# bowang-lab/BioReason

Hardware: AMD Instinct MI355X
Metric: GRPO samples/sec (NT-500M+Qwen3-1.7B, DNA 2x1024, prompt 2180, gen 256) (higher is better)
Workload: dtype bf16

## Files before the change

bioreason_amd/csrc/k_lora.hip:

```cpp
#include "bra_device.h"
#include "bra_api_internal.h"
#include "bra_lora_plan.h"

namespace bra {

struct LoraDownArgs {
    const bf16_t* x; long ldx;
    const bf16_t* A; long lda;
    bf16_t* t; long ldt;
    int M, K, R;
    float alpha;
    DropCfg d;
    int nb_live;
    int steps_per;
    float* part;
};

template <int RB, int NL, int TR = 32, int NT = NL>
__global__ __launch_bounds__(256) void lora_down_drop_kernel(LoraDownArgs g) {
    static_assert(TR == 8 || TR == 16 || TR == 32 || TR == 64 || TR == 128, "adapter ranks with dropout");
    static_assert(NL == (NT * TR + 31) / 32 && NL <= RB && NT <= 4, "live blocks = the blocks the targets cover");
    constexpr int KS = 128, XP = KS + 8;
    constexpr int XS_ELEMS = 2 * 32 * XP, AS_ELEMS = 2 * 32 * NL * XP;
    constexpr int RED_BYTES = 3 * NL * 64 * 16 * 4, STAGE_BYTES = (XS_ELEMS + AS_ELEMS) * 2;
    __shared__ __attribute__((aligned(16))) char lds[STAGE_BYTES > RED_BYTES ? STAGE_BYTES : RED_BYTES];
    bf16_t* xs = reinterpret_cast<bf16_t*>(lds);
    bf16_t* as = xs + XS_ELEMS;
    float* red = reinterpret_cast<float*>(lds);
    const int tid = (int)threadIdx.x, lane = tid & 63, wave = tid >> 6, h = lane >> 5;
    const int m0 = (int)blockIdx.x * 32;
    const int nstep = (g.K + KS - 1) / KS;
    const u32x4 zero4 = {0u, 0u, 0u, 0u};
    u32x4 rx[2], ra[2 * NL];
    auto issue = [&](int s) {
#pragma unroll
        for (int i = 0; i < 2; ++i) {
            const int c = tid + 256 * i, row = c >> 4, k = KS * s + 8 * (c & 15);
            int m = m0 + row; m = m < g.M ? m : g.M - 1;
            rx[i] = ld16(g.x + (long)m * g.ldx + (k < g.K ? k : 0));
        }
#pragma unroll
        for (int i = 0; i < 2 * NL; ++i) {
            const int c = tid + 256 * i, row = c >> 4, k = KS * s + 8 * (c & 15);
            ra[i] = ld16(g.A + (long)(row < g.R ? row : g.R - 1) * g.lda + (k < g.K ? k : 0));
        }
    };
    auto commit = [&](int buf, int s) {
#pragma unroll
        for (int i = 0; i < 2; ++i) {
            const int c = tid + 256 * i, k = KS * s + 8 * (c & 15);
            st16(&xs[buf * 32 * XP + (c >> 4) * XP + 8 * (c & 15)], k < g.K ? rx[i] : zero4);
        }
#pragma unroll
        for (int i = 0; i < 2 * NL; ++i) {
            const int c = tid + 256 * i, row = c >> 4, k = KS * s + 8 * (c & 15);
            st16(&as[buf * 32 * NL * XP + (c >> 4) * XP + 8 * (c & 15)], (k < g.K && row < g.R) ? ra[i] : zero4);
        }
    };
    f32x16 acc[NL];
#pragma unroll
    for (int rb = 0; rb < NL; ++rb)
#pragma unroll
        for (int q = 0; q < 16; ++q) acc[rb][q] = 0.f;
    const int s_lo = (int)blockIdx.y * g.steps_per;
    const int s_hi = s_lo + g.steps_per < nstep ? s_lo + g.steps_per : nstep;
    issue(s_lo); commit(s_lo & 1, s_lo);
    __syncthreads();
    const int mrow = m0 + (lane & 31);
    for (int s = s_lo; s < s_hi; ++s) {
        const int buf = s & 1;
        issue(s + 1 < s_hi ? s + 1 : s);
        sched_fence();
        const int lrow = opaque_i(lane & 31);
#pragma unroll
        for (int k2 = 0; k2 < 2; ++k2) {
            const int kk = 2 * wave + k2;
            const u32x4 xf = ld16(&xs[buf * 32 * XP + lrow * XP + 16 * kk + 8 * h]);
            const uint32_t e0 = (uint32_t)mrow * (uint32_t)g.K + (uint32_t)(KS * s + 16 * kk + 8 * h);
            if constexpr (TR == 32) {
#pragma unroll
                for (int rb = 0; rb < NL; ++rb) {
                    const u32x4 af = drop_apply8(xf, g.d.seed[rb], e0, g.d.thr16, g.d.inv_keep);
                    const u32x4 bf = ld16(&as[buf * 32 * NL * XP + (32 * rb + lrow) * XP + 16 * kk + 8 * h]);
                    acc[rb] = mfma_32x32x16(af, bf, acc[rb]);
                }
            } else if constexpr (TR > 32) {
#pragma unroll
                for (int jt = 0; jt < NT; ++jt) {
                    const u32x4 af = drop_apply8(xf, g.d.seed[jt], e0, g.d.thr16, g.d.inv_keep);
#pragma unroll
                    for (int b = 0; b < TR / 32; ++b) {
                        const int rb = jt * (TR / 32) + b;
                        const u32x4 bf = ld16(&as[buf * 32 * NL * XP + (32 * rb + lrow) * XP + 16 * kk + 8 * h]);
                        acc[rb] = mfma_32x32x16(af, bf, acc[rb]);
                    }
                }
            } else {
#pragma unroll
                for (int jt = 0; jt < NT; ++jt) {
                    const int rb = jt * TR / 32;
                    const u32x4 af = drop_apply8(xf, g.d.seed[jt], e0, g.d.thr16, g.d.inv_keep);
                    const u32x4 bf = ld16(&as[buf * 32 * NL * XP + (32 * rb + lrow) * XP + 16 * kk + 8 * h]);
                    acc[rb] = mfma_32x32x16(af, lrow / TR == jt % (32 / TR) ? bf : zero4, acc[rb]);
                }
            }
        }
        if (s + 1 < s_hi) commit(buf ^ 1, s + 1);
        __syncthreads();
    }
    if (wave != 0) {
#pragma unroll
        for (int rb = 0; rb < NL; ++rb)
#pragma unroll
            for (int q = 0; q < 16; ++q) red[(((wave - 1) * NL + rb) * 64 + lane) * 16 + q] = acc[rb][q];
    }
    __syncthreads();
    if (wave != 0) return;
    float* const pbase = g.part ? g.part + ((long)blockIdx.y * g.M + m0 + 4 * h) * g.R + (lane & 31) : nullptr;
    bf16_t* const tbase = g.t ? g.t + (long)(m0 + 4 * h) * g.ldt + (lane & 31) : nullptr;
#pragma unroll
    for (int rb = 0; rb < RB; ++rb) {
        const int r = 32 * rb + (lane & 31);
#pragma unroll
        for (int q = 0; q < 16; ++q) {
            const int mq = (q & 3) + 8 * (q >> 2);
            const int m = m0 + mq + 4 * h;
            float v = 0.f;
            if (rb < NL) {
                v = acc[rb < NL ? rb : 0][q];
#pragma unroll
                for (int w = 0; w < 3; ++w) v += red[((w * NL + (rb < NL ? rb : 0)) * 64 + lane) * 16 + q];
            }
            if (m < g.M && r < g.R) {
                if (g.part) pbase[(long)mq * g.R + 32 * rb] = v;
                else tbase[(long)mq * g.ldt + 32 * rb] = f2bf(g.alpha * v);
            }
        }
    }
}

__global__ __launch_bounds__(256) void lora_partial_reduce_kernel(const float* part, int ks, long MR, int R, float alpha, bf16_t* t, long ldt) {
    const long i4 = ((long)blockIdx.x * 256 + threadIdx.x) * 4;
    if (i4 >= MR) return;
    float a0 = 0.f, a1 = 0.f, a2 = 0.f, a3 = 0.f;
    for (int k = 0; k < ks; ++k) {
        const f32x4 v = *reinterpret_cast<const f32x4*>(part + (long)k * MR + i4);
        a0 += v[0]; a1 += v[1]; a2 += v[2]; a3 += v[3];
    }
    const long m = i4 / R;
    const int r = (int)(i4 - m * R);
    bf16_t* o = t + m * ldt + r;
    o[0] = f2bf(alpha * a0); o[1] = f2bf(alpha * a1); o[2] = f2bf(alpha * a2); o[3] = f2bf(alpha * a3);
}

struct LoraUpArgs {
    const bf16_t* dts; long ldd;
    const bf16_t* AT; long ldat;
    bf16_t* out; long ldo;
    int M, K, R;
    int k_chunk;
    DropCfg d;
    int nb_live;
};

template <int RB, int NL, int TR = 32, int NT = NL>
__global__ __launch_bounds__(256) void lora_up_drop_kernel(LoraUpArgs g) {
    constexpr int NC = TR == 32 ? 2 * NL : (NT * TR + 15) / 16;
    const u32x4 zero4 = {0u, 0u, 0u, 0u};
    const int lane = lane_id(), wave = (int)threadIdx.x >> 6, h = lane >> 5;
    const int m_base = ((int)blockIdx.x * 4 + wave) * 32;
    if (m_base >= g.M) return;
    int mr = m_base + (lane & 31); mr = mr < g.M ? mr : g.M - 1;
    u32x4 df[NC];
#pragma unroll
    for (int c = 0; c < NC; ++c) df[c] = ld16(g.dts + (long)mr * g.ldd + 16 * c + 8 * h);
    uint32_t rowbase[8];
    {
        const uint32_t odd0 = (uint32_t)lane & 1u;
#pragma unroll
        for (int i = 0; i < 8; ++i) {
            const int q = (int)(8 * odd0) + i;
            rowbase[i] = (uint32_t)(m_base + (q & 3) + 8 * (q >> 2) + 4 * h) * (uint32_t)g.K;
        }
    }
    const int k_lo = (int)blockIdx.y * g.k_chunk;
    int k_hi = k_lo + g.k_chunk; k_hi = k_hi < g.K ? k_hi : g.K;
    constexpr int UP_SP = 64 + 8;
    __shared__ __attribute__((aligned(16))) bf16_t stage[4][32 * UP_SP];
    bf16_t* sw = stage[wave];
    const bool vec_ok = !(g.ldo & 7) && !((size_t)g.out & 15) && !(k_lo & 7);
    for (int k0 = k_lo; k0 < k_hi; k0 += 32) {
        const int kc = k0 + (lane & 31);
        const int kr = kc < g.K ? kc : g.K - 1;
        u32x4 af[NC];
#pragma unroll
        for (int c = 0; c < NC; ++c) af[c] = ld16(g.AT + (long)kr * g.ldat + 16 * c + 8 * h);
        float o[16];
#pragma unroll
        for (int q = 0; q < 16; ++q) o[q] = 0.f;
        const uint32_t odd = (uint32_t)kr & 1u;
        const uint32_t fsh = odd ? 17u : 1u;
#pragma unroll
        for (int rb = 0; rb < NT; ++rb) {
            f32x16 acc;
#pragma unroll
            for (int q = 0; q < 16; ++q) acc[q] = 0.f;
            if constexpr (TR >= 16) {
#pragma unroll
                for (int c = rb * (TR / 16); c < (rb + 1) * (TR / 16); ++c) acc = mfma_32x32x16(df[c], af[c], acc);
            } else {
                acc = mfma_32x32x16(h == rb % 2 ? df[rb / 2] : zero4, af[rb / 2], acc);
            }
            uint32_t hh[16];
#pragma unroll
            for (int i = 0; i < 8; ++i) {
                const uint32_t mine = drop_hash(g.d.seed[rb], (rowbase[i] + (uint32_t)kr) >> 1);
                const uint32_t other = lane_swap1(mine);
                hh[i] = odd ? other : mine;
                hh[8 + i] = odd ? mine : other;
            }
#pragma unroll
            for (int q = 0; q < 16; ++q) o[q] += ((hh[q] >> fsh) & 0x7fffu) >= g.d.thr16 ? acc[q] : 0.f;
        }
        const int side = ((k0 - k_lo) >> 5) & 1;
#pragma unroll
        for (int q = 0; q < 16; ++q)
            sw[((q & 3) + 8 * (q >> 2) + 4 * h) * UP_SP + 32 * side + (lane & 31)] = kc < g.K ? f2bf(o[q] * g.d.inv_keep) : (bf16_t)0;
        if (side == 1 || k0 + 32 >= k_hi) {
            wave_lds_sync();
            const int kf = k0 - 32 * side;
            const int ncol = 32 * (side + 1);
#pragma unroll
            for (int j = 0; j < 4; ++j) {
                const int row = 8 * j + (lane >> 3), c8 = 8 * (lane & 7);
                const int m = m_base + row;
                const u32x4 v = ld16(&sw[row * UP_SP + c8]);
                if (m < g.M && c8 < ncol) {
                    bf16_t* op = g.out + (long)m * g.ldo + kf + c8;
                    if (vec_ok && kf + c8 + 8 <= g.K) st16(op, v);
                    else {
                        const bf16_t* e = reinterpret_cast<const bf16_t*>(&v);
                        for (int i = 0; i < 8; ++i) if (kf + c8 + i < g.K) op[i] = e[i];
                    }
                }
            }
            wave_lds_sync();
        }
    }
}

__global__ __launch_bounds__(256) void dropout_mask_kernel(uint8_t* out, long n, uint32_t seed, uint32_t thr16) {
    for (long i = (long)blockIdx.x * 256 + threadIdx.x; i < n; i += (long)gridDim.x * 256)
        out[i] = drop_keep1(seed, (uint32_t)i, thr16) ? 1 : 0;
}

}

using namespace bra;

extern "C" int bra_lora_down_splitk_plan(int M, int K) {
    const int gx = (M + 31) / 32, nstep = (K + 127) / 128;
    if (gx >= 192) return nstep >= 32 ? 4 : 1;
    if (gx <= 0 || nstep < 6) return 1;
    int want = 512 / gx, cap = nstep / 3;
    int ks = want < cap ? want : cap;
    if (ks < 2) return 1;
    const int per = (nstep + ks - 1) / ks;
    return (nstep + per - 1) / per;
}

extern "C" int bra_lora_down_drop(const void* x, long ldx, const void* A, long lda, void* t, long ldt, int M, int K, int R,
                                  float alpha, float p, unsigned s0, unsigned s1, unsigned s2, unsigned s3, int r, int nt,
                                  float* part, int ksplit, void* stream) {
    if (M == 0) return 0;
    if (!x || !A || !t || M < 0 || K <= 0 || K % 8 || ldx % 8 || lda % 8 || !lora_drop_ok(p, M, K, r, nt, R)) return BRA_ERR_ARG;
    if (ksplit <= 1) part = nullptr;
    else if (!part || ksplit > (K + 127) / 128 || ldt % 4) return BRA_ERR_ARG;
    const unsigned seeds[4] = {s0, s1, s2, s3};
    const int nstep = (K + 127) / 128;
    const int per = part ? (nstep + ksplit - 1) / ksplit : nstep;
    const int ny = part ? (nstep + per - 1) / per : 1;
    const dim3 grid((M + 31) / 32, ny);
    bra_stream_t st = (bra_stream_t)stream;
    return lora_for_slices(r, nt, R, [&](const LoraSlice& s) {
        float* const ps = part ? part + (long)ksplit * M * s.c0 : nullptr;
        bf16_t* const ts = (bf16_t*)t + s.c0;
        LoraDownArgs g = {(const bf16_t*)x, ldx, (const bf16_t*)A + (long)s.c0 * lda, lda, ts, ldt, M, K, s.Rs, alpha,
                          make_cfg(p, seeds + s.j0, s.nts), 0, per, ps};
#define BRA_LD(C_, RB_, NL_, TR_, NT_) if (C_) BRA_LAUNCH((lora_down_drop_kernel<RB_, NL_, TR_, NT_>), grid, dim3(256), 0, st, g); else
        BRA_LORA_ROWS(BRA_LD) return BRA_ERR_ARG;
#undef BRA_LD
        if (part) {
            const long MR = (long)M * s.Rs;
            BRA_LAUNCH(lora_partial_reduce_kernel, dim3((unsigned)((MR / 4 + 255) / 256)), dim3(256), 0, st, (const float*)ps, ny, MR, s.Rs,
                       alpha, ts, ldt);
        }
        return BRA_LAUNCH_STATUS();
    });
}

extern "C" int bra_lora_up_drop(const void* dts, long ldd, const void* AT, long ldat, void* out, long ldo, int M, int K, int R,
                                float p, unsigned s0, unsigned s1, unsigned s2, unsigned s3, int r, int nt, void* stream) {
    if (M == 0) return 0;
    if (!dts || !AT || !out || M < 0 || K <= 0 || ldd % 8 || ldat % 8 || !lora_drop_ok(p, M, K, r, nt, R)) return BRA_ERR_ARG;
    const int mblk = (M + 127) / 128;
    int splits = (1024 + mblk - 1) / mblk;
    int k_chunk = ((K + splits - 1) / splits + 31) / 32 * 32;
    k_chunk = k_chunk < 128 ? 128 : k_chunk;
    const unsigned seeds[4] = {s0, s1, s2, s3};
    LoraUpArgs g = {(const bf16_t*)dts, ldd, (const bf16_t*)AT, ldat, (bf16_t*)out, ldo, M, K, R, k_chunk, make_cfg(p, seeds, nt), 0};
    const dim3 grid(mblk, (K + k_chunk - 1) / k_chunk);
    bra_stream_t st = (bra_stream_t)stream;
#define BRA_LU(RB_, NL_, TR_, NT_) BRA_LAUNCH((lora_up_drop_kernel<RB_, NL_, TR_, NT_>), grid, dim3(256), 0, st, g)
#define BRA_LUR(TR_, NT_) BRA_LU((NT_ * TR_ + 63) / 64 * 2, (NT_ * TR_ + 31) / 32, TR_, NT_)
#define BRA_LUR3(TR_) do { if (nt == 1) BRA_LUR(TR_, 1); else if (nt == 2) BRA_LUR(TR_, 2); else BRA_LUR(TR_, 3); } while (0)
    if (r == 32 && R == 32) BRA_LU(1, 1, 32, 1);
    else if (r == 32 && R == 64) { if (nt == 1) BRA_LU(2, 1, 32, 1); else BRA_LU(2, 2, 32, 2); }
    else if (r == 32 && nt == 3) BRA_LU(4, 3, 32, 3);
    else if (r == 32) BRA_LU(4, 4, 32, 4);
    else if (r == 8) BRA_LUR3(8);
    else if (r == 16) BRA_LUR3(16);
    else if (r == 64) BRA_LUR3(64);
    else BRA_LUR3(128);
#undef BRA_LUR3
#undef BRA_LUR
#undef BRA_LU
    return BRA_LAUNCH_STATUS();
}

extern "C" int bra_dropout_mask(void* out, int M, int K, float p, unsigned seed, void* stream) {
    if (M <= 0 || K <= 0) return 0;
    if (!out || !(p >= 0.f && p < 1.f) || (long)M * K >= (1l << 32)) return BRA_ERR_ARG;
    const long n = (long)M * K;
    long grid = (n + 255) / 256; grid = grid > 4096 ? 4096 : grid;
    BRA_LAUNCH(dropout_mask_kernel, dim3((unsigned)grid), dim3(256), 0, (bra_stream_t)stream, (uint8_t*)out, n, (uint32_t)seed,
               drop_threshold(p));
    return BRA_LAUNCH_STATUS();
}
```

bioreason_amd/ops.py:

```python
from __future__ import annotations

import math
import os
from typing import Optional, Tuple

import torch

from ._lib import current_stream, get_lib

BF16 = torch.bfloat16


def _ld(t: torch.Tensor) -> int:
    assert t.stride(-1) == 1, "last dim must be contiguous"
    return t.stride(-2) if t.dim() >= 2 else t.shape[-1]


def _rows(t: torch.Tensor) -> int:
    return t.numel() // t.shape[-1]


def _as2d(t: torch.Tensor) -> torch.Tensor:
    return t.reshape(-1, t.shape[-1]) if t.dim() != 2 else t


def gemm_nt(
    a: torch.Tensor,
    b: torch.Tensor,
    *,
    a2: Optional[torch.Tensor] = None,
    b2: Optional[torch.Tensor] = None,
    bias: Optional[torch.Tensor] = None,
    res: Optional[torch.Tensor] = None,
    out: Optional[torch.Tensor] = None,
    alpha: float = 1.0,
    out_f32: bool = False,
    accumulate: bool = False,
) -> torch.Tensor:
    a = _as2d(a)
    M, K = a.shape
    N = b.shape[0]
    assert b.shape[1] == K and a.dtype == BF16 and b.dtype == BF16
    K2 = 0
    if a2 is not None:
        a2 = _as2d(a2)
        K2 = a2.shape[1]
        assert b2 is not None and b2.shape == (N, K2) and a2.shape[0] == M
    if out is None:
        out = torch.empty((M, N), dtype=torch.float32 if out_f32 else BF16, device=a.device)
    else:
        assert out.shape == (M, N) and out.dtype == (torch.float32 if out_f32 else BF16)
    if res is not None:
        res = _as2d(res)
        assert res.shape == (M, N) and res.dtype == BF16
    prof = GEMM_PROFILE
    timed = prof is not None and a.is_cuda and prof.wants(M, N, K, K2)
    if timed:
        e0 = torch.cuda.Event(enable_timing=True)
        e0.record()
    get_lib().call(
        "bra_gemm_bf16_nt", a, _ld(a), b, _ld(b), a2, _ld(a2) if a2 is not None else 0, b2,
        _ld(b2) if b2 is not None else 0, K2, out, _ld(out), M, N, K, alpha, bias, res,
        _ld(res) if res is not None else 0, int(out_f32), int(accumulate), current_stream(a),
    )
    if timed:
        e1 = torch.cuda.Event(enable_timing=True)
        e1.record()
        nbytes = 2.0 * (M * K + N * K + (M + N) * K2 + (M * N if res is not None else 0)) + M * N * (4.0 if out_f32 else 2.0)
        prof.records.append((2.0 * M * N * (K + K2), e0, e1, nbytes, (M, N, K, K2, res is not None)))
    return out


class GemmProfile:

    def __init__(self, min_m: int = 1024, dominant_only: bool = True):
        self.min_m = min_m
        self.dominant_only = dominant_only
        self.records = []

    def wants(self, M: int, N: int, K: int, K2: int) -> bool:
        if not self.dominant_only:
            return M >= self.min_m
        if K % 64 or K2 % 64:
            return False
        t = ((M + 255) // 256) * ((N + 255) // 256)
        rounds = (t + 255) // 256
        if t >= 140 and (t <= 256 or 100 * t >= 75 * rounds * 256):
            return True
        if ((M + 255) // 256) * ((N + 127) // 128) >= 128:
            return True
        return ((M + 127) // 128) * ((N + 127) // 128) >= 128

    def summary(self):
        torch.cuda.synchronize()
        fl = sum(r[0] for r in self.records)
        ms = sum(r[1].elapsed_time(r[2]) for r in self.records)
        n = len(self.records)
        by = sum(r[3] for r in self.records)
        return {"launches": n, "flops": fl, "ms": ms, "avg_launch_ms": ms / max(n, 1), "tflops": fl / max(ms, 1e-9) / 1e9,
                "flops_per_launch": fl / max(n, 1), "bytes_per_launch": by / max(n, 1)}


def gemm_profile_by_shape(prof: "GemmProfile"):
    torch.cuda.synchronize()
    agg = {}
    for r in prof.records:
        a = agg.setdefault(r[4], [0, 0.0, 0.0])
        a[0] += 1
        a[1] += r[1].elapsed_time(r[2])
        a[2] += r[0]
    return sorted(((k, n, ms, fl / max(ms, 1e-9) / 1e9) for k, (n, ms, fl) in agg.items()), key=lambda t: -t[2])


GEMM_PROFILE: Optional[GemmProfile] = None


def gemm_nt_splitk(a: torch.Tensor, b: torch.Tensor, out: torch.Tensor, alpha: float = 1.0, split_k: int = 0) -> torch.Tensor:
    M, K = a.shape
    N = b.shape[0]
    assert b.shape[1] == K and out.shape == (M, N) and out.dtype == torch.float32
    if split_k <= 0:
        tiles = ((M + 127) // 128) * ((N + 127) // 128)
        split_k = max(1, min(K // 256 if K >= 256 else 1, (512 + tiles - 1) // tiles))
    get_lib().call("bra_gemm_bf16_nt_splitk", a, _ld(a), b, _ld(b), out, _ld(out), M, N, K, alpha, split_k, current_stream(a))
    return out


def wgrad_tn(y: torch.Tensor, t: torch.Tensor, out: torch.Tensor, transposed_out: bool = False, alpha: float = 1.0,
             m_chunk: int = 0, drop=None, rank: int = 32) -> torch.Tensor:
    M, N = y.shape
    R = t.shape[1]
    assert t.shape[0] == M and out.dtype == torch.float32 and out.shape == ((R, N) if transposed_out else (N, R))
    c_sn, c_sr = (1, _ld(out)) if transposed_out else (_ld(out), 1)
    if drop is not None:
        get_lib().call("bra_wgrad_tn_drop", y, _ld(y), t, _ld(t), out, c_sn, c_sr, M, N, R, alpha, m_chunk, drop[0],
                       *_group(drop[1], rank, R), current_stream(y))
        return out
    get_lib().call("bra_wgrad_tn", y, _ld(y), t, _ld(t), out, c_sn, c_sr, M, N, R, alpha, m_chunk, current_stream(y))
    return out


LORA_DROP_RANKS = (8, 16, 32, 64, 128)


def _group(seeds, rank, R):
    if rank not in LORA_DROP_RANKS:
        raise NotImplementedError(f"LoRA dropout is built for adapter ranks {list(LORA_DROP_RANKS)}, not r = {rank}")
    if rank == 32:
        seeds = seeds[:max(R // 32, 1)]
    elif not 1 <= len(seeds) <= 3:
        raise ValueError(f"a fused LoRA group has 1 to 3 targets, got {len(seeds)} seeds")
    s = [int(x) & 0xFFFFFFFF for x in seeds]
    return (*(s + [0, 0, 0, 0])[:4], rank, len(s))


def dropout_mask(M: int, K: int, p: float, seed: int, device) -> torch.Tensor:
    out = torch.empty((M, K), dtype=torch.uint8, device=device)
    get_lib().call("bra_dropout_mask", out, M, K, p, int(seed) & 0xFFFFFFFF, current_stream(out))
    return out


LORA_DOWN_SPLITK = os.environ.get("BRA_LORA_SPLITK", "1") != "0"


def lora_down_drop(x: torch.Tensor, A: torch.Tensor, alpha: float, p: float, seeds, rank: int = 32) -> torch.Tensor:
    M, K = x.shape
    R = A.shape[0]
    t = torch.empty((M, R), dtype=BF16, device=x.device)
    lib = get_lib()
    ks = int(lib._dll.bra_lora_down_splitk_plan(int(M), int(K))) if LORA_DOWN_SPLITK else 1
    part = torch.empty((ks, M, R), dtype=torch.float32, device=x.device) if ks > 1 else None
    lib.call("bra_lora_down_drop", x, _ld(x), A, _ld(A), t, _ld(t), M, K, R, alpha, p, *_group(seeds, rank, R), part, ks,
             current_stream(x))
    return t


def lora_up_drop(dts: torch.Tensor, AT: torch.Tensor, p: float, seeds, rank: int = 32) -> torch.Tensor:
    M, R = dts.shape
    K = AT.shape[0]
    out = torch.empty((M, K), dtype=BF16, device=dts.device)
    get_lib().call("bra_lora_up_drop", dts, _ld(dts), AT, _ld(AT), out, _ld(out), M, K, R, p, *_group(seeds, rank, R),
                   current_stream(dts))
    return out


def lmhead_logprob(h: torch.Tensor, emb: torch.Tensor, tgt: torch.Tensor) -> Tuple[torch.Tensor, torch.Tensor]:
    M, K = h.shape
    V = emb.shape[0]
    nchunk = (V + 63) // 64
    dev = h.device
    pm = torch.empty((M, nchunk), dtype=torch.float32, device=dev)
    ps = torch.empty((M, nchunk), dtype=torch.float32, device=dev)
    tl = torch.zeros((M,), dtype=torch.float32, device=dev)
    lse = torch.empty((M,), dtype=torch.float32, device=dev)
    logp = torch.empty((M,), dtype=torch.float32, device=dev)
    st = current_stream(h)
    lib = get_lib()
    lib.call("bra_lmhead_lse_partials", h, _ld(h), emb, _ld(emb), M, V, K, tgt, pm, ps, tl, st)
    lib.call("bra_lse_merge", pm, ps, tl, lse, logp, M, nchunk, st)
    return logp, lse


def lmhead_dlogits(h: torch.Tensor, emb: torch.Tensor, tgt: torch.Tensor, lse: torch.Tensor, coef: torch.Tensor) -> torch.Tensor:
    M, K = h.shape
    V = emb.shape[0]
    out = torch.empty((M, V), dtype=BF16, device=h.device)
    get_lib().call("bra_lmhead_dlogits", h, _ld(h), emb, _ld(emb), M, V, K, tgt, lse, coef, out, _ld(out), current_stream(h))
    return out


def rmsnorm_fwd(x: torch.Tensor, w: torch.Tensor, eps: float) -> torch.Tensor:
    x2 = _as2d(x)
    y = torch.empty_like(x2)
    get_lib().call("bra_rmsnorm_fwd", x2, _ld(x2), w, y, _ld(y), None, x2.shape[0], x2.shape[1], eps, current_stream(x))
    return y.view(x.shape)


def rmsnorm_bwd(dy: torch.Tensor, x: torch.Tensor, w: torch.Tensor, eps: float, dres: Optional[torch.Tensor] = None) -> torch.Tensor:
    x2, dy2 = _as2d(x), _as2d(dy)
    dx = torch.empty_like(x2)
    d2 = _as2d(dres) if dres is not None else None
    get_lib().call("bra_rmsnorm_bwd", dy2, _ld(dy2), x2, _ld(x2), w, d2, _ld(d2) if d2 is not None else 0, dx, _ld(dx),
                   x2.shape[0], x2.shape[1], eps, current_stream(x))
    return dx.view(x.shape)


def layernorm_fwd(x: torch.Tensor, w: torch.Tensor, b: torch.Tensor, eps: float) -> torch.Tensor:
    x2 = _as2d(x)
    y = torch.empty_like(x2)
    get_lib().call("bra_layernorm_fwd", x2, _ld(x2), w, b, y, _ld(y), x2.shape[0], x2.shape[1], eps, current_stream(x))
    return y.view(x.shape)


def gemm_swiglu(x: torch.Tensor, W: torch.Tensor, a2: Optional[torch.Tensor] = None, b2: Optional[torch.Tensor] = None) -> Optional[torch.Tensor]:
    M, K = x.shape
    F = W.shape[0] // 2
    K2 = a2.shape[1] if a2 is not None else 0
    if M <= 16 or K % 64 or K2 % 64 or F % 128 or W.shape[0] != 2 * F:
        return None
    act = torch.empty((M, F), dtype=BF16, device=x.device)
    rc = get_lib().call_rc("bra_gemm_swiglu_bf16_nt", x, _ld(x), W, _ld(W), a2, _ld(a2) if a2 is not None else 0, b2,
                           _ld(b2) if b2 is not None else 0, K2, act, _ld(act), M, F, K, 1.0, current_stream(x))
    return None if rc != 0 else act


def swiglu_fwd(gu: torch.Tensor) -> torch.Tensor:
    gu2 = _as2d(gu)
    F = gu2.shape[1] // 2
    act = torch.empty((gu2.shape[0], F), dtype=BF16, device=gu.device)
    get_lib().call("bra_swiglu_fwd", gu2, _ld(gu2), act, _ld(act), gu2.shape[0], F, current_stream(gu))
    return act


def swiglu_bwd(gu: torch.Tensor, dact: torch.Tensor) -> torch.Tensor:
    gu2, d2 = _as2d(gu), _as2d(dact)
    F = gu2.shape[1] // 2
    dgu = torch.empty_like(gu2)
    get_lib().call("bra_swiglu_bwd", gu2, _ld(gu2), d2, _ld(d2), dgu, _ld(dgu), gu2.shape[0], F, current_stream(gu))
    return dgu


def _bsh_strides(t: torch.Tensor) -> Tuple[int, int, int]:
    assert t.dim() == 4 and t.stride(3) == 1
    return t.stride(0), t.stride(1), t.stride(2)


def qk_norm_rope_fwd(qkv, qw, kw, cosT, sinT, pos, S, Hq, Hkv, hd, eps, qscale, q, k, v, s_off=0):
    T = qkv.shape[0]
    get_lib().call("bra_qk_norm_rope_fwd", qkv, _ld(qkv), qw, kw, cosT, sinT, pos, T, S, Hq, Hkv, hd, eps, qscale,
                   q, *_bsh_strides(q), k, *_bsh_strides(k), v, *_bsh_strides(v), s_off, current_stream(qkv))


def qk_norm_rope_bwd(qkv, qw, kw, cosT, sinT, pos, S, Hq, Hkv, hd, eps, qscale, dq, dk, dv):
    T = qkv.shape[0]
    dqkv = torch.empty_like(qkv)
    get_lib().call("bra_qk_norm_rope_bwd", qkv, _ld(qkv), qw, kw, cosT, sinT, pos, T, S, Hq, Hkv, hd, eps, qscale,
                   dq, *_bsh_strides(dq), dk, *_bsh_strides(dk), dv, *_bsh_strides(dv), dqkv, _ld(dqkv), current_stream(qkv))
    return dqkv


def pad64(n: int) -> int:
    return (n + 63) // 64 * 64


def head_transpose(x: torch.Tensor) -> torch.Tensor:
    B, S, H, hd = x.shape
    out = torch.empty((B, H, hd, pad64(S)), dtype=BF16, device=x.device)
    sb, ss, sh = _bsh_strides(x)
    get_lib().call("bra_head_transpose", x, sb, ss, sh, out, out.stride(0), out.stride(1), out.stride(2), B, S, H, hd, current_stream(x))
    return out


def attn_fwd(q, k, vt, kmask, causal: bool, scale: float, q_off: Optional[int] = None, need_lse: bool = True,
             out: Optional[torch.Tensor] = None, nsplit: Optional[int] = None):
    B, Sq, Hq, hd = q.shape
    Sk, Hkv = k.shape[1], k.shape[2]
    if q_off is None:
        q_off = Sk - Sq
    o = out if out is not None else torch.empty((B, Sq, Hq, hd), dtype=BF16, device=q.device)
    lse = torch.empty((B, Hq, Sq), dtype=torch.float32, device=q.device) if need_lse else None
    ns = attn_fwd_split_parts(B, Hq, Sq, Sk, hd, causal) if nsplit is None else int(nsplit)
    if ns > 1:
        part_o = torch.empty((B, Hq, ns, Sq, hd), dtype=torch.float32, device=q.device)
        part_ml = torch.empty((B, Hq, ns, Sq, 2), dtype=torch.float32, device=q.device)
        get_lib().call("bra_attn_fwd_split", q, *_bsh_strides(q), k, *_bsh_strides(k), vt, vt.stride(0), vt.stride(1), vt.stride(2),
                       o, *_bsh_strides(o), lse, kmask, B, Hq, Hkv, Sq, Sk, hd, int(causal), q_off, scale, ns, part_o, part_ml,
                       current_stream(q))
        return o, lse
    get_lib().call("bra_attn_fwd", q, *_bsh_strides(q), k, *_bsh_strides(k), vt, vt.stride(0), vt.stride(1), vt.stride(2),
                   o, *_bsh_strides(o), lse, kmask, B, Hq, Hkv, Sq, Sk, hd, int(causal), q_off, scale, current_stream(q))
    return o, lse


ATTN_SPLIT = os.environ.get("BRA_ATTN_SPLIT", "1") == "1"


def attn_fwd_split_parts(B: int, Hq: int, Sq: int, Sk: int, hd: int, causal: bool) -> int:
    if not ATTN_SPLIT or hd < 64 or Sq <= 128 or Sk < 1024:
        return 1
    wgs = ((Sq + 255) // 256) * Hq * B
    if wgs >= 200:
        return 1
    return max(1, min(4, (300 + wgs // 2) // wgs))


def attn_bwd_split_parts(B: int, Hq: int, Hkv: int, Sq: int, Sk: int, hd: int, causal: bool):
# ... 385 lines not shown
```

include/bioreason_hip.h:

```cpp
#ifndef BIOREASON_HIP_H
#define BIOREASON_HIP_H
#ifdef __cplusplus
extern "C" {
#endif

#define BRA_ERR_ARG (-1)
#define BRA_ERR_UNSUPPORTED (-2)

int bra_gemm_bf16_nt(const void* A, long lda, const void* B, long ldb, const void* A2, long lda2, const void* B2,
                     long ldb2, int K2, void* C, long ldc, int M, int N, int K, float alpha, const void* bias,
                     const void* res, long ldres, int out_f32, int accumulate, void* stream);

int bra_gemm_bf16_nt_splitk(const void* A, long lda, const void* B, long ldb, void* C, long ldc, int M, int N, int K,
                            float alpha, int split_k, void* stream);

int bra_wgrad_tn(const void* Y, long ldy, const void* T, long ldt, float* C, long c_sn, long c_sr, int M, int N, int R,
                 float alpha, int m_chunk, void* stream);

int bra_lora_down_splitk_plan(int M, int K);
int bra_lora_down_drop(const void* x, long ldx, const void* A, long lda, void* t, long ldt, int M, int K, int R, float alpha,
                       float p, unsigned s0, unsigned s1, unsigned s2, unsigned s3, int r, int nt, float* part, int ksplit,
                       void* stream);
int bra_lora_up_drop(const void* dts, long ldd, const void* AT, long ldat, void* out, long ldo, int M, int K, int R, float p,
                     unsigned s0, unsigned s1, unsigned s2, unsigned s3, int r, int nt, void* stream);
int bra_wgrad_tn_drop(const void* Y, long ldy, const void* T, long ldt, float* C, long c_sn, long c_sr, int M, int N, int R,
                      float alpha, int m_chunk, float p, unsigned s0, unsigned s1, unsigned s2, unsigned s3, int r, int nt,
                      void* stream);
int bra_dropout_mask(void* out, int M, int K, float p, unsigned seed, void* stream);

int bra_lmhead_lse_partials(const void* H, long ldh, const void* E, long lde, int M, int V, int K, const int* tgt,
                            float* part_max, float* part_sum, float* tgt_logit, void* stream);
int bra_lse_merge(const float* part_max, const float* part_sum, const float* tgt_logit, float* lse, float* logp,
                  int rows, int nchunk, void* stream);
int bra_lmhead_dlogits(const void* H, long ldh, const void* E, long lde, int M, int V, int K, const int* tgt,
                       const float* lse, const float* coef, void* dlogits, long ldd, void* stream);

int bra_rmsnorm_fwd(const void* x, long ldx, const void* w, void* y, long ldy, float* rstd, int rows, int cols,
                    float eps, void* stream);
int bra_rmsnorm_bwd(const void* dy, long lddy, const void* x, long ldx, const void* w, const void* dres, long lddres,
                    void* dx, long lddx, int rows, int cols, float eps, void* stream);
int bra_layernorm_fwd(const void* x, long ldx, const void* w, const void* b, void* y, long ldy, int rows, int cols,
                      float eps, void* stream);
int bra_swiglu_fwd(const void* gu, long ldgu, void* act, long ldact, int rows, int F, void* stream);
int bra_swiglu_bwd(const void* gu, long ldgu, const void* dact, long lddact, void* dgu, long lddgu, int rows, int F,
                   void* stream);
int bra_qk_norm_rope_fwd(const void* qkv, long ldqkv, const void* qw, const void* kw, const float* cosT,
                         const float* sinT, const int* pos, int T, int S, int Hq, int Hkv, int hd, float eps,
                         float qscale, void* q, long q_sb, long q_ss, long q_sh, void* k, long k_sb, long k_ss,
                         long k_sh, void* v, long v_sb, long v_ss, long v_sh, int s_off, void* stream);
int bra_qk_norm_rope_bwd(const void* qkv, long ldqkv, const void* qw, const void* kw, const float* cosT,
                         const float* sinT, const int* pos, int T, int S, int Hq, int Hkv, int hd, float eps,
                         float qscale, const void* dq, long q_sb, long q_ss, long q_sh, const void* dk, long k_sb,
                         long k_ss, long k_sh, const void* dv, long v_sb, long v_ss, long v_sh, void* dqkv,
                         long lddqkv, void* stream);

int bra_attn_fwd(const void* q, long q_sb, long q_ss, long q_sh, const void* k, long k_sb, long k_ss, long k_sh,
                 const void* vt, long vt_sb, long vt_sh, long vt_sd, void* o, long o_sb, long o_ss, long o_sh,
                 float* lse, const void* kmask, int B, int Hq, int Hkv, int Sq, int Sk, int hd, int causal,
                 int q_off, float scale, void* stream);
int bra_attn_fwd_split(const void* q, long q_sb, long q_ss, long q_sh, const void* k, long k_sb, long k_ss, long k_sh,
                       const void* vt, long vt_sb, long vt_sh, long vt_sd, void* o, long o_sb, long o_ss, long o_sh,
                       float* lse, const void* kmask, int B, int Hq, int Hkv, int Sq, int Sk, int hd, int causal,
                       int q_off, float scale, int nsplit, float* part_o, float* part_ml, void* stream);
int bra_attn_bwd(const void* q, long q_sb, long q_ss, long q_sh, const void* k, long k_sb, long k_ss, long k_sh,
                 const void* v, long v_sb, long v_ss, long v_sh, const void* dout, long do_sb, long do_ss, long do_sh,
                 const void* kt, long kt_sb, long kt_sh, long kt_sd, const void* qt, long qt_sb, long qt_sh,
                 long qt_sd, const void* dot, long dot_sb, long dot_sh, long dot_sd, const float* lse,
                 const float* delta, const void* kmask, void* dq, long dq_sb, long dq_ss, long dq_sh, void* dk,
                 long dk_sb, long dk_ss, long dk_sh, void* dv, long dv_sb, long dv_ss, long dv_sh, int B, int Hq,
                 int Hkv, int Sq, int Sk, int hd, int causal, int q_off, float scale, void* stream);
int bra_attn_bwd_split(const void* q, long q_sb, long q_ss, long q_sh, const void* k, long k_sb, long k_ss, long k_sh,
                 const void* v, long v_sb, long v_ss, long v_sh, const void* dout, long do_sb, long do_ss, long do_sh,
                 const void* kt, long kt_sb, long kt_sh, long kt_sd, const void* qt, long qt_sb, long qt_sh,
                 long qt_sd, const void* dot, long dot_sb, long dot_sh, long dot_sd, const float* lse,
                 const float* delta, const void* kmask, void* dq, long dq_sb, long dq_ss, long dq_sh, void* dk,
                 long dk_sb, long dk_ss, long dk_sh, void* dv, long dv_sb, long dv_ss, long dv_sh, int B, int Hq,
                 int Hkv, int Sq, int Sk, int hd, int causal, int q_off, float scale, int nsplit_dq, float* part_dq, int nsplit_kv, float* part_dk, float* part_dv, void* stream);
int bra_attn_decode_nchunk(int len);
int bra_attn_decode(const void* q, const void* kc, const void* vc, const void* kmask, float* part_o, float* part_ml,
                    void* o, int B, int Hq, int Hkv, int hd, int Smax, int len, float scale, void* stream);

int bra_qwen_layer_desc_size(void);
int bra_qwen_decode_step(const void* layers_host, int L, int B, int H, int Hq, int Hkv, int hd, int F, int Smax,
                         float eps, float scale, const void* E, const void* norm_w, const float* cosT,
                         const float* sinT, const int* tok, const int* pos, const void* kmask, int cur_len,
                         int lora_on, void* x, void* xn, void* qkv, void* q, void* o, void* h, void* hn, void* gu,
                         void* act, void* t, float* part_o, float* part_ml, void* hid, void* stream);

int bra_dec_gemm(const void* x, long ldx, const void* norm_w, float eps, const void* W, long ldw, const void* res,
                 long ldres, void* out, long ldo, int M, int N, int K, int act, int out_f32, void* stream);
int bra_dec_attn_partial(const void* qkv, long ldqkv, const void* qw, const void* kw, const float* cosT,
                         const float* sinT, const int* pos, void* kc, void* vc, const void* kmask, float* part_o,
                         float* part_ml, int B, int Hq, int Hkv, int hd, int Smax, int cur_len, float eps, float scale,
                         int chunk_off, int nchunk_tot, const int* t_dev, void* stream);
int bra_dec_gemm2(const void* x, long ldx, const float* ss_in, int nss_in, const void* norm_w, float eps, const void* W,
                  long ldw, const void* res, long ldres, void* out, long ldo, float* ss_out, int nss_out, int M, int N,
                  int K, int act, int out_f32, void* stream);
int bra_dec_gemm2_packed(const void* x, long ldx, const float* ss_in, int nss_in, const void* norm_w, float eps, const void* W,
                         long ldw, const void* res, long ldres, void* out, long ldo, float* ss_out, int nss_out, int M, int N,
                         int K, int act, int out_f32, int packed, void* stream);
int bra_dec_pack_weights_fp8(const void* W, long ldw, int N, int K, int act, int out_f32, const void* norm_w, void* out_q,
                             float* out_scale, void* stream);
int bra_dec_gemm2_fp8(const void* x, long ldx, const float* ss_in, int nss_in, float eps, const void* Wq, const float* wscale,
                      const void* res, long ldres, void* out, long ldo, float* ss_out, int nss_out, int M, int N, int K, int act,
                      int out_f32, int norm_folded, void* stream);
int bra_gemm_swiglu_bf16_nt(const void* A, long lda, const void* W, long ldw, const void* A2, long lda2, const void* B2, long ldb2, int K2,
                            void* C, long ldc, int M, int F, int K, float alpha, void* stream);
int bra_quant_rows_fp8(const void* x, long ldx, int M, int K, const void* colw, void* q, long ldq, float* scale, int rms, float eps,
                       void* stream);
int bra_swiglu_quant_fp8(const void* gu, long ldgu, int M, int F, void* q, long ldq, float* scale, void* stream);
int bra_gemm_fp8_nt(const void* A8, long lda, const float* sa, const void* B8, long ldb, const float* sb, void* C, long ldc, int M, int N,
                    int K, const void* res, long ldres, int out_f32, void* stream);
int bra_dec_pack_weights(const void* W, long ldw, int N, int K, int act, int out_f32, const void* norm_w, void* out, void* stream);
int bra_dec_pack_weights_rows(const void* W, long ldw, int N, int K, int act, int out_f32, const void* norm_w, int rows, void* out,
                              void* stream);
int bra_row_sumsq(const void* x, long ldx, int M, int K, float* ss, int nss, void* stream);
int bra_dec_attn_shared(const void* qkv, long ldqkv, const void* qw, const float* cosT, const float* sinT, const int* pos,
                        const void* kp, long kp_sr, long kp_sh, long kp_ss, const void* vtp, long vt_sr, long vt_sh,
                        long vt_sd, const void* pmask, float* part_o, float* part_ml, int R, int copies, int Hq, int Hkv,
                        int hd, int P, int nchunk_tot, float eps, float scale, const int* t_dev, void* stream);
int bra_dec_attn_both(const void* qkv, long ldqkv, const void* qw, const void* kw, const float* cosT, const float* sinT,
                      const int* pos, const void* kp, long kp_sr, long kp_sh, long kp_ss, const void* vtp, long vt_sr,
                      long vt_sh, long vt_sd, const void* pmask, void* kc, void* vc, float* part_o, float* part_ml, int R,
                      int copies, int Hq, int Hkv, int hd, int P, int C, int t, float eps, float scale, const int* t_dev,
                      const float* rope_rows, void* stream);
int bra_attn_decode_merge(const float* part_o, const float* part_ml, void* o, int B, int Hq, int hd, int nchunk,
                          const int* t_dev, int npc, void* stream);
int bra_qwen_decode_step_fused(const void* layers_host, int L, int B, int H, int Hq, int Hkv, int hd, int F, int Smax,
                               int V, float eps, float scale, const void* E, const void* norm_w, const float* cosT,
                               const float* sinT, const int* tok, const int* pos, const void* kmask, int cur_len,
                               const int* len_dev, int embed_done, void* x, void* qkv, void* o, void* h, void* act, float* ss_ws,
                               int nss, float* part_o, float* part_ml, float* logits, void* stream);

int bra_qwen_decode_step_shared(const void* layers_host, int L, int R, int copies, int H, int Hq, int Hkv, int hd, int F,
                                int P, long vt_pitch, int C, int V, float eps, float scale, const void* E,
                                const void* norm_w, const float* cosT, const float* sinT, const int* tok, const int* pos,
                                const void* pmask, int t, const int* t_dev, int embed_done, void* x, void* qkv, void* o, void* h,
                                void* act, float* ss_ws, int nss, float* part_o, float* part_ml, float* logits, void* stream);

int bra_dec_attn_one(const void* qkv, long ldqkv, const void* qw, const void* kw, const float* cosT, const float* sinT,
                     const int* pos, const float* rope_rows, const void* kp, long kp_sr, long kp_sh, long kp_ss,
                     const void* vtp, long vt_sr, long vt_sh, long vt_sd, const void* pmask, void* kc, void* vct, long cp,
                     float* part_o, float* part_ml, int nslot, void* o, long ldo, int R, int copies,
                     int Hq, int Hkv, int hd, int P, int C, int t, float eps, float scale, const int* t_dev, void* stream);
int bra_qwen_decode_step_one(const void* layers_host, int L, int R, int copies, int H, int Hq, int Hkv, int hd, int F,
                             int P, long vt_pitch, int C, long cp, int V, float eps, float scale, const void* E,
                             const void* norm_w, const float* cosT, const float* sinT, const int* tok, const int* pos,
                             const void* pmask, int t, const int* t_dev, int embed_done, void* x, void* qkv, void* o, void* h,
                             void* act, float* ss_ws, int nss, float* part_o, float* part_ml, int nslot, float* logits,
                             void* stream);

int bra_head_transpose(const void* x, long sb, long ss, long sh, void* xt, long t_sb, long t_sh, long pitch, int B,
                       int S, int H, int hd, void* stream);
int bra_attn_delta(const void* dout, long do_sb, long do_ss, long do_sh, const void* o, long o_sb, long o_ss,
                   long o_sh, float* delta, int B, int S, int H, int hd, void* stream);
int bra_dna_scatter_plan(const int* ids, int ntok, int dna_id, const void* dna_mask, int nseq, int Sd,
                         const int* seq_order, int* tok_src, int* counts, void* stream);
int bra_embed_scatter_fwd(const int* ids, const int* tok_src, const void* E, long lde, const void* dna, long ldd,
                          void* out, long ldo, int ntok, int H, void* stream);
int bra_embed_scatter_bwd(const int* tok_src, const void* dout, long ldo, void* ddna, long ldd, int ntok, int H,
                          void* stream);
int bra_gather_rows(const int* rows, const void* x, long ldx, void* out, long ldo, int n, int H, void* stream);
int bra_scatter_rows(const int* rows, const void* x, long ldx, void* out, long ldo, int n, int H, void* stream);
int bra_transpose2d(const void* in, long ldi, void* out, long ldo, int rows, int cols, void* stream);
int bra_colsum(const void* x, long ldx, float* out, int rows, int cols, void* stream);
int bra_pack_desc_size(void);
int bra_pack_params(const void* descs_dev, int ndesc, long max_elems, void* stream);
int bra_vec_sum(const float* x, long n, float scale, float* out, void* stream);
int bra_cast_grad(const void* src, void* dst, long n, int to_f32, void* stream);
int bra_sumsq(const float* g, const void* mask, long n, float* out, float* ws, void* stream);
int bra_adamw(float* p, const float* g, float* m, float* v, const void* mask, long n, float lr, float b1, float b2,
              float eps, float wd, int step, const float* sumsq, float max_norm, float grad_scale, void* stream);
// ... 48 lines not shown
```

include/bioreason_hip_debug.h:

```cpp
#ifndef BIOREASON_HIP_DEBUG_H
#define BIOREASON_HIP_DEBUG_H
#include "bioreason_hip.h"
#ifdef __cplusplus
extern "C" {
#endif

int bra_gemm_set_variant(int v);
int bra_gemm_set_ring_fill(int pct);
int bra_gemm_set_row_split(int on);
int bra_gemm_set_epi_lds(int on);
int bra_sample_set_one_launch(int on);
int bra_gemm_set_glds_rows(int rows);
int bra_attn_set_block_order(int legacy);
int bra_attn_set_fwd4(int on);
int bra_attn_set_bwd4(int mask);
int bra_attn_set_probe(void* buf);


int bra_dec_gemm2_probe(const void* x, long ldx, const float* ss_in, int nss_in, const void* norm_w, float eps, const void* W,
                        long ldw, const void* res, long ldres, void* out, long ldo, float* ss_out, int nss_out, int M, int N,
                        int K, int act, int out_f32, int packed, void* probe, void* stream);
int bra_debug_set_probe(void* p);

int bra_gridsync_bytes(void);
int bra_persist_layer_desc_size(void);
int bra_persist_set_stamps(void* p);
int bra_qwen_layers_persist(const void* layers_dev, int L, int R, int copies, int H, int Hq, int Hkv, int hd, int F, int P,
                            long vt_pitch, int C, long cp, float eps, float scale, const float* cosT, const float* sinT,
                            const int* pos, const float* rope_rows, const void* pmask, int t, const int* t_dev, void* x,
                            void* qkv, void* o, void* h, void* act, float* ss_ws, int nss, float* part_o, float* part_ml,
                            int nslot, void* sync, int prefetch, int stop_after, int timeout_us, void* stream);
int bra_qwen_decode_step_persist(const void* layers_host, const void* layers_dev, int L, int R, int copies, int H, int Hq, int Hkv,
                                 int hd, int F, int P, long vt_pitch, int C, long cp, int V, float eps, float scale, const void* E,
                                 const void* norm_w, const float* cosT, const float* sinT, const int* tok, const int* pos,
                                 const void* pmask, int t, const int* t_dev, int embed_done, void* x, void* qkv, void* o, void* h,
                                 void* act, float* ss_ws, int nss, float* part_o, float* part_ml, int nslot, float* logits,
                                 void* sync, int prefetch, int stop_after, int timeout_us, void* stream);
int bra_chain_probe(void* done, void* buf, void* errs, const void* wts, long wts_bytes, int nwg, int n, int chained, int wchunks,
                    int timeout_us, void* stream_a, void* stream_b);
int bra_gridbar_probe(void* sync, void* buf, void* errs, const void* wts, long wts_bytes, int nwg, int iters, int mode,
                      int wchunks, int timeout_us, void* stream);

#ifdef __cplusplus
}
#endif
#endif
```

Measured before the change: 19.61.

## Fuse split-K LoRA-down reduction via ticket counter and deepen global prefetch

The LoRA-down dropout kernel now keeps a two-deep register prefetch set, so loads for step s+2 are issued while step s computes. Split-K partial sums are reduced inside the kernel: each block bumps a per-tile ticket, and the last block to arrive sums all slices and writes bf16 output. This removes the separate partial-reduce launch and its extra pass over the partials. It costs more registers, needs cross-block atomics and memory fences, and relies on a persistent ticket buffer that must be reset to zero after each use.

```diff
diff --git a/bioreason_amd/csrc/k_lora.hip b/bioreason_amd/csrc/k_lora.hip
--- a/bioreason_amd/csrc/k_lora.hip
+++ b/bioreason_amd/csrc/k_lora.hip
@@ -1,6 +1,8 @@
 #include "bra_device.h"
 #include "bra_api_internal.h"
 #include "bra_lora_plan.h"
+#include "bra_gridsync.h"
+#include <type_traits>
 
 namespace bra {
 
@@ -11,9 +13,9 @@
     int M, K, R;
     float alpha;
     DropCfg d;
-    int nb_live;
     int steps_per;
     float* part;
+    unsigned* tickets;
 };
 
 template <int RB, int NL, int TR = 32, int NT = NL>
@@ -31,30 +33,32 @@
     const int m0 = (int)blockIdx.x * 32;
     const int nstep = (g.K + KS - 1) / KS;
     const u32x4 zero4 = {0u, 0u, 0u, 0u};
-    u32x4 rx[2], ra[2 * NL];
-    auto issue = [&](int s) {
+    u32x4 rx[2][2], ra[2][2 * NL];
+    auto issue = [&](auto set, int s) {
+        constexpr int q = decltype(set)::value;
 #pragma unroll
         for (int i = 0; i < 2; ++i) {
             const int c = tid + 256 * i, row = c >> 4, k = KS * s + 8 * (c & 15);
             int m = m0 + row; m = m < g.M ? m : g.M - 1;
-            rx[i] = ld16(g.x + (long)m * g.ldx + (k < g.K ? k : 0));
+            rx[q][i] = ld16(g.x + (long)m * g.ldx + (k < g.K ? k : 0));
         }
 #pragma unroll
         for (int i = 0; i < 2 * NL; ++i) {
             const int c = tid + 256 * i, row = c >> 4, k = KS * s + 8 * (c & 15);
-            ra[i] = ld16(g.A + (long)(row < g.R ? row : g.R - 1) * g.lda + (k < g.K ? k : 0));
+            ra[q][i] = ld16(g.A + (long)(row < g.R ? row : g.R - 1) * g.lda + (k < g.K ? k : 0));
         }
     };
-    auto commit = [&](int buf, int s) {
+    auto commit = [&](auto set, int buf, int s) {
+        constexpr int q = decltype(set)::value;
 #pragma unroll
         for (int i = 0; i < 2; ++i) {
             const int c = tid + 256 * i, k = KS * s + 8 * (c & 15);
-            st16(&xs[buf * 32 * XP + (c >> 4) * XP + 8 * (c & 15)], k < g.K ? rx[i] : zero4);
+            st16(&xs[buf * 32 * XP + (c >> 4) * XP + 8 * (c & 15)], k < g.K ? rx[q][i] : zero4);
         }
 #pragma unroll
         for (int i = 0; i < 2 * NL; ++i) {
             const int c = tid + 256 * i, row = c >> 4, k = KS * s + 8 * (c & 15);
-            st16(&as[buf * 32 * NL * XP + (c >> 4) * XP + 8 * (c & 15)], (k < g.K && row < g.R) ? ra[i] : zero4);
+            st16(&as[buf * 32 * NL * XP + (c >> 4) * XP + 8 * (c & 15)], (k < g.K && row < g.R) ? ra[q][i] : zero4);
         }
     };
     f32x16 acc[NL];
@@ -64,12 +68,16 @@
         for (int q = 0; q < 16; ++q) acc[rb][q] = 0.f;
     const int s_lo = (int)blockIdx.y * g.steps_per;
     const int s_hi = s_lo + g.steps_per < nstep ? s_lo + g.steps_per : nstep;
-    issue(s_lo); commit(s_lo & 1, s_lo);
+    const std::integral_constant<int, 0> set0;
+    const std::integral_constant<int, 1> set1;
+    issue(set0, s_lo);
+    issue(set1, s_lo + 1 < s_hi ? s_lo + 1 : s_lo);
+    commit(set0, s_lo & 1, s_lo);
     __syncthreads();
     const int mrow = m0 + (lane & 31);
-    for (int s = s_lo; s < s_hi; ++s) {
+    auto kstep = [&](int s, auto mine, auto more) {
         const int buf = s & 1;
-        issue(s + 1 < s_hi ? s + 1 : s);
+        if constexpr (decltype(more)::value) issue(mine, s + 2 < s_hi ? s + 2 : s);
         sched_fence();
         const int lrow = opaque_i(lane & 31);
 #pragma unroll
@@ -105,9 +113,23 @@
                 }
             }
         }
-        if (s + 1 < s_hi) commit(buf ^ 1, s + 1);
+    };
+    int s = s_lo;
+    for (; s + 2 < s_hi; s += 2) {
+        kstep(s, set0, std::true_type());
+        commit(set1, (s + 1) & 1, s + 1);
         __syncthreads();
-    }
+        kstep(s + 1, set1, std::true_type());
+        commit(set0, s & 1, s + 2);
+        __syncthreads();
+    }
+    kstep(s, set0, std::false_type());
+    if (s + 1 < s_hi) {
+        commit(set1, (s + 1) & 1, s + 1);
+        __syncthreads();
+        kstep(s + 1, set1, std::false_type());
+    }
+    __syncthreads();
     if (wave != 0) {
 #pragma unroll
         for (int rb = 0; rb < NL; ++rb)
@@ -115,27 +137,102 @@
             for (int q = 0; q < 16; ++q) red[(((wave - 1) * NL + rb) * 64 + lane) * 16 + q] = acc[rb][q];
     }
     __syncthreads();
-    if (wave != 0) return;
-    float* const pbase = g.part ? g.part + ((long)blockIdx.y * g.M + m0 + 4 * h) * g.R + (lane & 31) : nullptr;
-    bf16_t* const tbase = g.t ? g.t + (long)(m0 + 4 * h) * g.ldt + (lane & 31) : nullptr;
-#pragma unroll
-    for (int rb = 0; rb < RB; ++rb) {
-        const int r = 32 * rb + (lane & 31);
-#pragma unroll
-        for (int q = 0; q < 16; ++q) {
-            const int mq = (q & 3) + 8 * (q >> 2);
-            const int m = m0 + mq + 4 * h;
-            float v = 0.f;
-            if (rb < NL) {
-                v = acc[rb < NL ? rb : 0][q];
-#pragma unroll
-                for (int w = 0; w < 3; ++w) v += red[((w * NL + (rb < NL ? rb : 0)) * 64 + lane) * 16 + q];
-            }
-            if (m < g.M && r < g.R) {
-                if (g.part) pbase[(long)mq * g.R + 32 * rb] = v;
-                else tbase[(long)mq * g.ldt + 32 * rb] = f2bf(g.alpha * v);
-            }
-        }
+    const bool fused = g.part != nullptr && g.tickets != nullptr;
+    if (wave != 0 && !fused) return;
+    float* const pslab = g.part ? g.part + (long)blockIdx.y * g.M * g.R : nullptr;
+    if (wave == 0) {
+        const long pidx = (long)(m0 + 4 * h) * g.R + (lane & 31);
+        float* const pbase = g.part ? pslab + pidx : nullptr;
+        const unsigned poff = (unsigned)(pidx * 4);
+        bf16_t* const tbase = g.t ? g.t + (long)(m0 + 4 * h) * g.ldt + (lane & 31) : nullptr;
+        auto tile_out = [&](auto put) {
+#pragma unroll
+            for (int rb = 0; rb < RB; ++rb) {
+                const int r = 32 * rb + (lane & 31);
+#pragma unroll
+                for (int q = 0; q < 16; ++q) {
+                    const int mq = (q & 3) + 8 * (q >> 2);
+                    const int m = m0 + mq + 4 * h;
+                    float v = 0.f;
+                    if (rb < NL) {
+#pragma clang fp reassociate(off)
+                        v = acc[rb < NL ? rb : 0][q];
+#pragma unroll
+                        for (int w = 0; w < 3; ++w) v = v + red[((w * NL + (rb < NL ? rb : 0)) * 64 + lane) * 16 + q];
+                    }
+                    if (m < g.M && r < g.R) put(mq, rb, v);
+                }
+            }
+        };
+        if (fused) tile_out([&](int mq, int rb, float v) { xst4f<1>(pslab, poff + (unsigned)((mq * g.R + 32 * rb) * 4), v); });
+        else if (g.part) tile_out([&](int mq, int rb, float v) { pbase[(long)mq * g.R + 32 * rb] = v; });
+        else tile_out([&](int mq, int rb, float v) { tbase[(long)mq * g.ldt + 32 * rb] = f2bf(g.alpha * v); });
+        if (!fused) return;
+#ifndef BRA_EMU
+        gs_drain();
+#endif
+    }
+    unsigned* const flag = reinterpret_cast<unsigned*>(lds);
+    __syncthreads();
+    if (tid == 0) {
+#ifndef BRA_EMU
+        *flag = gs_add(g.tickets + blockIdx.x, 1u);
+#else
+        *flag = atomicAdd(g.tickets + blockIdx.x, 1u);
+#endif
+    }
+    __syncthreads();
+    if (*flag != gridDim.y - 1u) return;
+    const int ny = (int)gridDim.y;
+    const long MR = (long)g.M * g.R;
+    const int cpr = g.R >> 2;
+    f32x4 a[RB];
+    unsigned off[RB];
+    bool live[RB];
+#pragma unroll
+    for (int c = 0; c < RB; ++c) {
+        const int ci = tid + 256 * c, row = ci / cpr, col = 4 * (ci - row * cpr);
+        live[c] = row < 32 && m0 + row < g.M;
+        off[c] = live[c] ? (unsigned)(((long)(m0 + row) * g.R + col) * 4) : 0u;
+#pragma unroll
+        for (int e = 0; e < 4; ++e) a[c][e] = 0.f;
+    }
+    for (int k0 = 0; k0 < ny; k0 += 4) {
+        u32x4 v[4][RB];
+#pragma unroll
+        for (int j = 0; j < 4; ++j)
+            if (k0 + j < ny) {
+#pragma unroll
+                for (int c = 0; c < RB; ++c) v[j][c] = xld16<1>(g.part + (long)(k0 + j) * MR, off[c]);
+            }
+        {
+#pragma clang fp reassociate(off)
+#pragma unroll
+            for (int j = 0; j < 4; ++j)
+                if (k0 + j < ny) {
+#pragma unroll
+                    for (int c = 0; c < RB; ++c) {
+                        const f32x4 f = __builtin_bit_cast(f32x4, v[j][c]);
+#pragma unroll
+                        for (int e = 0; e < 4; ++e) a[c][e] = a[c][e] + f[e];
+                    }
+                }
+        }
+    }
+#pragma unroll
+    for (int c = 0; c < RB; ++c) {
+        if (!live[c]) continue;
+        const int ci = tid + 256 * c, row = ci / cpr, col = 4 * (ci - row * cpr);
+        bf16_t* o = g.t + (long)(m0 + row) * g.ldt + col;
+#pragma unroll
+        for (int e = 0; e < 4; ++e) o[e] = f2bf(g.alpha * a[c][e]);
+    }
+    if (tid == 0) {
+#ifndef BRA_EMU
+        gs_store(g.tickets + blockIdx.x, 0u);
+#else
+        g.tickets[blockIdx.x] = 0u;
+#endif
     }
 }
 
@@ -269,9 +366,18 @@
     return (nstep + per - 1) / per;
 }
 
-extern "C" int bra_lora_down_drop(const void* x, long ldx, const void* A, long lda, void* t, long ldt, int M, int K, int R,
-                                  float alpha, float p, unsigned s0, unsigned s1, unsigned s2, unsigned s3, int r, int nt,
-                                  float* part, int ksplit, void* stream) {
+#ifdef BRA_DEBUG
+#ifdef BRA_EMU
+static int g_lora_down_two_launch = 0;
+#else
+static std::atomic<int> g_lora_down_two_launch(0);
+#endif
+extern "C" int bra_lora_down_set_two_launch(int on) { g_lora_down_two_launch = on ? 1 : 0; return 0; }
+#endif
+
+extern "C" int bra_lora_down_drop_tk(const void* x, long ldx, const void* A, long lda, void* t, long ldt, int M, int K, int R,
+                                     float alpha, float p, unsigned s0, unsigned s1, unsigned s2, unsigned s3, int r, int nt,
+                                     float* part, int ksplit, unsigned* tickets, void* stream) {
     if (M == 0) return 0;
     if (!x || !A || !t || M < 0 || K <= 0 || K % 8 || ldx % 8 || lda % 8 || !lora_drop_ok(p, M, K, r, nt, R)) return BRA_ERR_ARG;
     if (ksplit <= 1) part = nullptr;
@@ -282,21 +388,31 @@
     const int ny = part ? (nstep + per - 1) / per : 1;
     const dim3 grid((M + 31) / 32, ny);
     bra_stream_t st = (bra_stream_t)stream;
+#ifdef BRA_DEBUG
+    if (g_lora_down_two_launch) tickets = nullptr;
+#endif
+    if (!part || (long)M * 128 * 4 >= (1l << 31)) tickets = nullptr;
     return lora_for_slices(r, nt, R, [&](const LoraSlice& s) {
         float* const ps = part ? part + (long)ksplit * M * s.c0 : nullptr;
         bf16_t* const ts = (bf16_t*)t + s.c0;
         LoraDownArgs g = {(const bf16_t*)x, ldx, (const bf16_t*)A + (long)s.c0 * lda, lda, ts, ldt, M, K, s.Rs, alpha,
-                          make_cfg(p, seeds + s.j0, s.nts), 0, per, ps};
+                          make_cfg(p, seeds + s.j0, s.nts), per, ps, tickets ? tickets + (long)(s.c0 / 128) * grid.x : nullptr};
 #define BRA_LD(C_, RB_, NL_, TR_, NT_) if (C_) BRA_LAUNCH((lora_down_drop_kernel<RB_, NL_, TR_, NT_>), grid, dim3(256), 0, st, g); else
         BRA_LORA_ROWS(BRA_LD) return BRA_ERR_ARG;
 #undef BRA_LD
-        if (part) {
+        if (part && !tickets) {
             const long MR = (long)M * s.Rs;
             BRA_LAUNCH(lora_partial_reduce_kernel, dim3((unsigned)((MR / 4 + 255) / 256)), dim3(256), 0, st, (const float*)ps, ny, MR, s.Rs,
                        alpha, ts, ldt);
         }
         return BRA_LAUNCH_STATUS();
     });
+}
+
+extern "C" int bra_lora_down_drop(const void* x, long ldx, const void* A, long lda, void* t, long ldt, int M, int K, int R,
+                                  float alpha, float p, unsigned s0, unsigned s1, unsigned s2, unsigned s3, int r, int nt,
+                                  float* part, int ksplit, void* stream) {
+    return bra_lora_down_drop_tk(x, ldx, A, lda, t, ldt, M, K, R, alpha, p, s0, s1, s2, s3, r, nt, part, ksplit, nullptr, stream);
 }
 
 extern "C" int bra_lora_up_drop(const void* dts, long ldd, const void* AT, long ldat, void* out, long ldo, int M, int K, int R,
diff --git a/bioreason_amd/ops.py b/bioreason_amd/ops.py
--- a/bioreason_amd/ops.py
+++ b/bioreason_amd/ops.py
@@ -163,15 +163,31 @@
 LORA_DOWN_SPLITK = os.environ.get("BRA_LORA_SPLITK", "1") != "0"
 
 
+_LORA_TICKETS = {}
+
+
+def _lora_tickets(x: torch.Tensor, stream: int, words: int) -> torch.Tensor:
+    key = (x.device, stream)
+    buf = _LORA_TICKETS.get(key)
+    if buf is None or buf.numel() < words:
+        buf = torch.zeros(max(words, 1024), dtype=torch.int32, device=x.device)
+        _LORA_TICKETS[key] = buf
+    return buf
+
+
 def lora_down_drop(x: torch.Tensor, A: torch.Tensor, alpha: float, p: float, seeds, rank: int = 32) -> torch.Tensor:
     M, K = x.shape
     R = A.shape[0]
     t = torch.empty((M, R), dtype=BF16, device=x.device)
     lib = get_lib()
     ks = int(lib._dll.bra_lora_down_splitk_plan(int(M), int(K))) if LORA_DOWN_SPLITK else 1
-    part = torch.empty((ks, M, R), dtype=torch.float32, device=x.device) if ks > 1 else None
-    lib.call("bra_lora_down_drop", x, _ld(x), A, _ld(A), t, _ld(t), M, K, R, alpha, p, *_group(seeds, rank, R), part, ks,
-             current_stream(x))
+    stream = current_stream(x)
+    part = tickets = None
+    if ks > 1:
+        part = torch.empty((ks, M, R), dtype=torch.float32, device=x.device)
+        tickets = _lora_tickets(x, stream, ((R + 127) // 128) * ((M + 31) // 32))
+    lib.call("bra_lora_down_drop_tk", x, _ld(x), A, _ld(A), t, _ld(t), M, K, R, alpha, p, *_group(seeds, rank, R), part, ks,
+             tickets, stream)
     return t
 
 
diff --git a/include/bioreason_hip.h b/include/bioreason_hip.h
--- a/include/bioreason_hip.h
+++ b/include/bioreason_hip.h
@@ -18,6 +18,9 @@
                  float alpha, int m_chunk, void* stream);
 
 int bra_lora_down_splitk_plan(int M, int K);
+int bra_lora_down_drop_tk(const void* x, long ldx, const void* A, long lda, void* t, long ldt, int M, int K, int R, float alpha,
+                          float p, unsigned s0, unsigned s1, unsigned s2, unsigned s3, int r, int nt, float* part, int ksplit,
+                          unsigned* tickets, void* stream);
 int bra_lora_down_drop(const void* x, long ldx, const void* A, long lda, void* t, long ldt, int M, int K, int R, float alpha,
                        float p, unsigned s0, unsigned s1, unsigned s2, unsigned s3, int r, int nt, float* part, int ksplit,
                        void* stream);
diff --git a/include/bioreason_hip_debug.h b/include/bioreason_hip_debug.h
--- a/include/bioreason_hip_debug.h
+++ b/include/bioreason_hip_debug.h
@@ -15,6 +15,7 @@
 int bra_attn_set_fwd4(int on);
 int bra_attn_set_bwd4(int mask);
 int bra_attn_set_probe(void* buf);
+int bra_lora_down_set_two_launch(int on);
 
 
 int bra_dec_gemm2_probe(const void* x, long ldx, const float* ss_in, int nss_in, const void* norm_w, float eps, const void* W,
```

Result: no change. 19.59 (-0.1%).
